# malani86/unet-DC-segmentation

Hardware: NVIDIA B200
Metric: images/sec end-to-end (mask + droplet table) (higher is better)
Workload: dtype bf16

## Files before the change

### include/unetdc_b200.h

```cpp
#ifndef UNETDC_B200_H
#define UNETDC_B200_H

#include <stddef.h>
#include <stdint.h>

#ifdef __cplusplus
extern "C" {
#endif

#define DC_OK 0
#define DC_EINVAL (-1)
#define DC_ECUDA (-2)
#define DC_EDEVICE (-3)
#define DC_ECAPACITY (-4)
#define DC_EWORKSPACE (-5)

#define DC_ABI_VERSION 205

const char* dc_last_error(void);
int dc_version(void);
int dc_device_check(int device, int* sm_count);

enum { DC_KIND_CONV3X3 = 0, DC_KIND_UPCONV2 = 1 };
enum {
    DC_EPI_STORE = 0,
    DC_EPI_STORE_POOL = 1,
    DC_EPI_HEAD = 2,
    DC_EPI_UPSCATTER = 3
};

typedef struct dc_conv_args {
    int kind;
    int epilogue;
    int relu;
    int B, H, W;
    int Cin, Cout;
    int dilation;
    const void* in;
    int in_stride;
    const void* weight;
    const float* bias;
    void* out;
    int out_stride;
    int out_offset;
    void* pool_out;
    int pool_stride;
    const float* head_w;
    float head_b;
    float thresh;
    float* prob_out;
    uint8_t* mask_out;
    const void* weight_par;
} dc_conv_args_t;

int dc_conv_tc(const dc_conv_args_t* args, void* stream);

typedef struct dc_upfuse_args {
    int B, H, W;
    const void* x;
    int x_stride;
    const void* skip;
    int skip_stride;
    const void* weight;
    const float* bias9;
    int relu;
    void* out;
    int out_stride;
    int out_offset;
    int channels;
    const void* weight_skip;
} dc_upfuse_args_t;

int dc_conv_upfused(const dc_upfuse_args_t* args, void* stream);
int dc_debug_upfuse_schedule(int* out, int cap);
int dc_debug_set_upfuse_mode(int mode);

enum { DC_CONV_FAMILY_AUTO = 0, DC_CONV_FAMILY_NO_PAIR = 1, DC_CONV_FAMILY_GENERIC = 2 };
int dc_debug_set_conv_family(int family);

typedef struct dc_stem_args {
    int in_kind;
    int B, H, W;
    int Cout;
    int dilation;
    const void* in;
    const float* weight;
    const float* bias;
    void* out;
    int out_stride;
    int out_offset;
} dc_stem_args_t;

int dc_stem(const dc_stem_args_t* args, void* stream);

typedef struct dc_model dc_model_t;

#define DC_NUM_LAYERS 23
typedef struct dc_model_desc {
    const void* weight[DC_NUM_LAYERS];
    const float* bias[DC_NUM_LAYERS];
    int dilations[5];
    int base_channels;
    int in_channels;
    int out_channels;
    const void* fused_weight1;
    const float* fused_bias1;
    const void* fused_wide_x[3];
    const void* fused_wide_s[3];
    const float* fused_wide_b[3];
    const void* par_weight[2];
} dc_model_desc_t;

int dc_model_create(dc_model_t** out, int device, const dc_model_desc_t* desc);
int dc_model_destroy(dc_model_t* m);
int dc_forward_workspace_bytes(const dc_model_t* m, int B, int H, int W, size_t* bytes);
int dc_forward(dc_model_t* m, int in_kind, const void* in, int B, int H, int W, float thresh, float* prob_out,
               uint8_t* mask_out, void* workspace, size_t workspace_bytes, void* stream);
int dc_forward_num_launches(const dc_model_t* m);
int dc_forward_profile(dc_model_t* m, int in_kind, const void* in, int B, int H, int W, float thresh, float* prob_out,
                       uint8_t* mask_out, void* workspace, size_t workspace_bytes, void* stream, float* launch_ms);

typedef struct dc_rolling_ball_args {
    const uint8_t* in;
    uint8_t* out;
    int B, H, W, C;
    int radius;
    void* workspace;
    size_t workspace_bytes;
} dc_rolling_ball_args_t;

// ... 96 lines not shown
```

### unet_dc_segmentation_b200/_lib.py

```python
from __future__ import annotations

import ctypes as C
from ctypes import POINTER, Structure, c_double, c_float, c_int, c_int32, c_int64, c_size_t, c_uint8, c_void_p

from . import build as _build

DC_OK = 0
DC_EINVAL, DC_ECUDA, DC_EDEVICE, DC_ECAPACITY, DC_EWORKSPACE = -1, -2, -3, -4, -5
DC_KIND_CONV3X3, DC_KIND_UPCONV2 = 0, 1
DC_EPI_STORE, DC_EPI_STORE_POOL, DC_EPI_HEAD, DC_EPI_UPSCATTER = 0, 1, 2, 3
DC_NUM_LAYERS = 23
DC_CONV_FAMILY_AUTO, DC_CONV_FAMILY_NO_PAIR, DC_CONV_FAMILY_GENERIC = 0, 1, 2
ABI_VERSION = 205

EXPORTS = [
    "dc_last_error", "dc_version", "dc_device_check", "dc_conv_tc", "dc_conv_upfused", "dc_debug_upfuse_schedule", "dc_debug_set_upfuse_mode", "dc_debug_set_conv_family", "dc_stem", "dc_model_create",
    "dc_model_destroy", "dc_forward_workspace_bytes", "dc_forward", "dc_forward_num_launches", "dc_forward_profile",
    "dc_rolling_ball_workspace_bytes", "dc_rolling_ball", "dc_rolling_ball_max_radius", "dc_debug_rolling_ball_plan", "dc_label_workspace_bytes", "dc_label_stats",
    "dc_resize_linear_u8", "dc_overlay_workspace_bytes", "dc_overlay_stencil",
    "dc_roi_workspace_bytes", "dc_roi_mask", "dc_radial_workspace_bytes", "dc_radial_density",
    "dc_spatial_workspace_bytes", "dc_spatial_density",
]


class DcError(RuntimeError):
    def __init__(self, code: int, msg: str):
        super().__init__(f"libunetdc_b200: {msg} (code {code})")
        self.code = code


class ConvArgs(Structure):
    _fields_ = [
        ("kind", c_int), ("epilogue", c_int), ("relu", c_int),
        ("B", c_int), ("H", c_int), ("W", c_int),
        ("Cin", c_int), ("Cout", c_int), ("dilation", c_int),
        ("in_", c_void_p), ("in_stride", c_int),
        ("weight", c_void_p), ("bias", c_void_p),
        ("out", c_void_p), ("out_stride", c_int), ("out_offset", c_int),
        ("pool_out", c_void_p), ("pool_stride", c_int),
        ("head_w", c_void_p), ("head_b", c_float), ("thresh", c_float),
        ("prob_out", c_void_p), ("mask_out", c_void_p),
        ("weight_par", c_void_p),
    ]


class StemArgs(Structure):
    _fields_ = [
        ("in_kind", c_int), ("B", c_int), ("H", c_int), ("W", c_int), ("Cout", c_int), ("dilation", c_int),
        ("in_", c_void_p), ("weight", c_void_p), ("bias", c_void_p), ("out", c_void_p),
        ("out_stride", c_int), ("out_offset", c_int),
    ]


class ModelDesc(Structure):
    _fields_ = [
        ("weight", c_void_p * DC_NUM_LAYERS), ("bias", c_void_p * DC_NUM_LAYERS),
        ("dilations", c_int * 5), ("base_channels", c_int), ("in_channels", c_int), ("out_channels", c_int),
        ("fused_weight1", c_void_p), ("fused_bias1", c_void_p),
        ("fused_wide_x", c_void_p * 3), ("fused_wide_s", c_void_p * 3), ("fused_wide_b", c_void_p * 3),
        ("par_weight", c_void_p * 2),
    ]


class UpfuseArgs(Structure):
    _fields_ = [
# ... 145 lines not shown
```

### unet_dc_segmentation_b200/csrc/conv_tc.cu

```cuda
#include "common.cuh"

#include <cuda.h>
#include <stdlib.h>
#include <string.h>

namespace dc {

namespace {

constexpr int TILE_H = 8, TILE_W = 16, TILE_M = TILE_H * TILE_W;
constexpr int KCHUNK = 64;
constexpr int A_STAGE_BYTES = TILE_M * KCHUNK * 2;
constexpr int NUM_THREADS = 384;
constexpr int EPI_WARP0 = 4;

int g_kernel_family = DC_CONV_FAMILY_AUTO;
int g_upfuse_mode = 0;

template <class K>
int set_max_smem_once(K kernel, int bytes, unsigned long long* done_mask) {
    int dev = 0;
    DC_CUDA(cudaGetDevice(&dev));
    const unsigned long long bit = 1ull << (dev & 63);
    if (!(__atomic_load_n(done_mask, __ATOMIC_ACQUIRE) & bit)) {
        DC_CUDA(cudaFuncSetAttribute(kernel, cudaFuncAttributeMaxDynamicSharedMemorySize, bytes));
        __atomic_fetch_or(done_mask, bit, __ATOMIC_RELEASE);
    }
    return DC_OK;
}

struct FastDiv {
    uint32_t mul, shift;
};
inline FastDiv make_fastdiv(int d) {
    FastDiv f;
    uint32_t s = 0;
    while ((1ll << s) < d) ++s;
    f.shift = 31 + s;
    f.mul = (uint32_t)(((1ull << f.shift) / (uint32_t)d) + 1ull);
    return f;
}
__device__ __forceinline__ int fast_div(int n, const FastDiv& f) {
    return (int)(((unsigned long long)(uint32_t)n * f.mul) >> f.shift);
}

struct alignas(64) ConvParams {
    CUtensorMap tmA;
    CUtensorMap tmB;
    CUtensorMap tmS;
    CUtensorMap tmB2;
    int B, H, W, Cin, Cout;
    int dil, ntaps, kchunks;
    int tiles_w, tiles_h, n_tiles, total_tiles, m_tiles;
    FastDiv fd_ntiles, fd_per_img, fd_tiles_w;
    int epilogue, relu;
    const float* bias;
    int bias_const;
    float bias_c[64];
    __nv_bfloat16* out;
    int out_stride, out_offset;
    __nv_bfloat16* pool_out;
    int pool_stride;
    const float* head_w;
    float head_b, thresh;
    float* prob_out;
    uint8_t* mask_out;
    int region_w, region_h, region_stride, nstages, nbstages;
    int border_bias;
    int real_ntiles;
};

struct TileCoord {
    int img, h0, w0, n0;
};

template <int TH = TILE_H, int TW = TILE_W>
__device__ __forceinline__ TileCoord decode_tile(const ConvParams& p, int tile, int BN) {
    TileCoord t;
    int m = fast_div(tile, p.fd_ntiles);
    int nt = tile - m * p.n_tiles;
    int per_img = p.tiles_h * p.tiles_w;
    t.img = fast_div(m, p.fd_per_img);
    int r = m - t.img * per_img;
    int th = fast_div(r, p.fd_tiles_w);
    t.h0 = th * TH;
    t.w0 = (r - th * p.tiles_w) * TW;
    t.n0 = nt * BN;
    return t;
}

template <int TH = TILE_H, int TW = TILE_W>
__device__ __forceinline__ bool tap_offset(const ConvParams& p, const TileCoord& t, int tap, int& dy, int& dx) {
    if (p.ntaps == 1) { dy = 0; dx = 0; return true; }
    int ky = tap / 3, kx = tap - ky * 3;
    dy = (ky - 1) * p.dil;
    dx = (kx - 1) * p.dil;
    return (t.h0 + dy + TH > 0) && (t.h0 + dy < p.H) && (t.w0 + dx + TW > 0) && (t.w0 + dx < p.W);
}

__device__ __forceinline__ uint32_t pack_bf16(float a, float b) {
    __nv_bfloat162 h = __floats2bfloat162_rn(a, b);
    return *reinterpret_cast<uint32_t*>(&h);
}
__device__ __forceinline__ uint32_t max_bf16x2(uint32_t a, uint32_t b) {
    __nv_bfloat162 r = __hmax2(*reinterpret_cast<__nv_bfloat162*>(&a), *reinterpret_cast<__nv_bfloat162*>(&b));
    return *reinterpret_cast<uint32_t*>(&r);
}

__device__ __forceinline__ int pair_count(const ConvParams& p) {
    return ((p.m_tiles + 1) >> 1) * p.n_tiles;
}
__device__ __forceinline__ int pair_to_tile(const ConvParams& p, int pair, int rank) {
    const int m_tiles = p.m_tiles;
    const int mpair = fast_div(pair, p.fd_ntiles), nt = pair - mpair * p.n_tiles;
    int m = 2 * mpair + rank;
    if (m >= m_tiles) m = m_tiles - 1;
    return m * p.n_tiles + nt;
}

__device__ __forceinline__ void tmem_ld_wait_on(uint32_t* v) {
    asm volatile("tcgen05.wait::ld.sync.aligned;"
                 : "+r"(v[0]), "+r"(v[1]), "+r"(v[2]), "+r"(v[3]), "+r"(v[4]), "+r"(v[5]), "+r"(v[6]), "+r"(v[7]),
                   "+r"(v[8]), "+r"(v[9]), "+r"(v[10]), "+r"(v[11]), "+r"(v[12]), "+r"(v[13]), "+r"(v[14]), "+r"(v[15]),
                   "+r"(v[16]), "+r"(v[17]), "+r"(v[18]), "+r"(v[19]), "+r"(v[20]), "+r"(v[21]), "+r"(v[22]), "+r"(v[23]),
                   "+r"(v[24]), "+r"(v[25]), "+r"(v[26]), "+r"(v[27]), "+r"(v[28]), "+r"(v[29]), "+r"(v[30]), "+r"(v[31])
                 :
                 : "memory");
}

constexpr int EPI_GROUPS = 2;
constexpr int EPI_STAGE_BYTES = 32 * 64;
constexpr int EPI_STAGE_TOTAL = EPI_GROUPS * 4 * EPI_STAGE_BYTES;

__device__ __forceinline__ uint32_t stg_off(int r, int q) {
    return (uint32_t)(((r >> 1) << 7) | (((r ^ (r >> 1)) & 1) << 6) | ((q ^ ((r >> 1) & 3)) << 4));
}

__device__ __forceinline__ uint32_t pack_bf16_relu(float a, float b) {
    uint32_t r;
    asm("cvt.rn.relu.bf16x2.f32 %0, %1, %2;" : "=r"(r) : "f"(b), "f"(a));
    return r;
}
template <bool PAIR>
__device__ __forceinline__ void release_accumulator(uint64_t* bar, int lane) {
    tc_fence_before();
    __syncwarp();
    if (lane == 0) {
        if (PAIR) mbar_arrive_leader(bar);
        else mbar_arrive(bar);
    }
}

template <int BN, int TH, int TW, int NHALF = 1, bool PAIR = false, bool COOP = true, bool UPF = false>
__device__ __forceinline__ void run_epilogue(const ConvParams& p, const int e, const int lane, const int group,
                                             const uint32_t tmem_base, uint64_t* tfull_bar, uint64_t* tempty_bar,
                                             const float* bias_s, uint8_t* stg_all) {
    const int L = e * 32 + lane;
    const int lh = L / TW, lw = L % TW;
    const float* head_s = bias_s + p.Cout;
    uint8_t* stg = stg_all + (group * 4 + e) * EPI_STAGE_BYTES;
    const int sq = lane & 3;
    const int pool_r0 = (TW == 16) ? 2 * (lane >> 2) : (16 * (lane >> 4) + 2 * ((lane >> 2) & 3));
    constexpr int CPG = COOP ? BN / 64 : BN / 32;
    constexpr int CSTEP = COOP ? 64 : 32;
    constexpr int NI = NHALF * CPG;
    const int cgrp = COOP ? group * 32 : 0;
    const bool up = !UPF && p.epilogue == DC_EPI_UPSCATTER;
// ... 265 lines not shown
                }
            }
        }
    } else if (warp == 1) {
        const uint32_t idesc = umma_idesc_bf16(TILE_M, BN);
        int stage = 0;
        uint32_t phase = 0;
        int it = 0;
        for (int tile = blockIdx.x; tile < p.total_tiles; tile += gridDim.x, ++it) {
            const TileCoord t = decode_tile(p, tile, BN);
            const int as = it & 1;
            const uint32_t aphase = (uint32_t)(it >> 1) & 1u;
            mbar_wait(&tempty_bar[as], aphase ^ 1u);
            tc_fence_after();
            const uint32_t d_tmem = tmem_base + (uint32_t)(as * BN);
            uint32_t accumulate = 0;
            for (int tap = 0; tap < p.ntaps; ++tap) {
                int dy, dx;
                if (!tap_offset(p, t, tap, dy, dx)) continue;
                for (int kc = 0; kc < p.kchunks; ++kc) {
                    mbar_wait(&full_bar[stage], phase);
                    tc_fence_after();
                    const uint32_t sa = smem_u32(smem + stage * STAGE_BYTES);
                    const uint64_t adesc = umma_desc_sw128(sa);
                    const uint64_t bdesc = umma_desc_sw128(sa + A_STAGE_BYTES);
                    if (elect_one()) {
#pragma unroll
                        for (int k = 0; k < KCHUNK / 16; ++k) {
                            umma_bf16(d_tmem, adesc + (uint64_t)(2 * k), bdesc + (uint64_t)(2 * k), idesc,
                                      (k == 0) ? accumulate : 1u);
                        }
                        umma_commit(&empty_bar[stage]);
                    }
                    __syncwarp();
                    accumulate = 1;
                    if (++stage == NSTAGES) { stage = 0; phase ^= 1u; }
                }
            }
            if (elect_one()) umma_commit(&tfull_bar[as]);
            __syncwarp();
        }
    } else if (warp >= EPI_WARP0) {
        run_epilogue<BN, TILE_H, TILE_W>(p, warp & 3, lane, (warp - EPI_WARP0) >> 2, tmem_base, tfull_bar, tempty_bar, bias_s, stg_s);
    }

    tc_fence_before();
    __syncthreads();
    if (warp == 2) {
        tc_fence_after();
        tmem_dealloc(tmem_base, TMEM_COLS);
    }
}

constexpr int HT_H = 16, HT_W = 8;
constexpr int HALO_MAX_STAGES = 8;
constexpr int HALO_BAR_BYTES = 512;
constexpr int HALO_BIAS_BYTES = 4096 + 256;

__device__ __forceinline__ uint64_t umma_desc_sw128_strided(uint32_t smem_addr, uint32_t sbo_bytes) {
    uint64_t d = 0;
    d |= (uint64_t)((smem_addr & 0x3FFFF) >> 4);
    d |= (uint64_t)1 << 16;
    d |= (uint64_t)((sbo_bytes >> 4) & 0x3FFF) << 32;
    d |= (uint64_t)1 << 46;
    d |= (uint64_t)2 << 61;
    return d;
}

template <int BN, int HT_NHALF, bool WRES>
__global__ void __launch_bounds__(NUM_THREADS, 1) conv_halo_kernel(const __grid_constant__ ConvParams p) {
    constexpr int HT_TW = HT_W * HT_NHALF;
    constexpr int W_TILE_BYTES = BN * KCHUNK * 2;
    constexpr int TMEM_COLS = 2 * HT_NHALF * BN;

    extern __shared__ uint8_t smem_raw[];
    uint8_t* smem = smem_raw + ((1024u - (smem_u32(smem_raw) & 1023u)) & 1023u);
    const int n_wtiles = WRES ? 9 * p.kchunks : p.nbstages;
    uint8_t* w_res = smem;
    uint8_t* a_ring = smem + n_wtiles * W_TILE_BYTES;
    uint64_t* full_bar = reinterpret_cast<uint64_t*>(a_ring + p.nstages * p.region_stride);
    uint64_t* empty_bar = full_bar + HALO_MAX_STAGES;
    uint64_t* bfull_bar = empty_bar + HALO_MAX_STAGES;
    uint64_t* bempty_bar = bfull_bar + HALO_MAX_STAGES;
    uint64_t* tfull_bar = bempty_bar + HALO_MAX_STAGES;
    uint64_t* tempty_bar = tfull_bar + 2;
    uint64_t* w_bar = tempty_bar + 2;
    uint32_t* tmem_slot = reinterpret_cast<uint32_t*>(w_bar + 1);
    float* bias_s = reinterpret_cast<float*>(reinterpret_cast<uint8_t*>(full_bar) + HALO_BAR_BYTES);
    uint8_t* stg_s = reinterpret_cast<uint8_t*>(full_bar) + HALO_BAR_BYTES + HALO_BIAS_BYTES;

    const int warp = threadIdx.x >> 5, lane = threadIdx.x & 31;
    const int NST = p.nstages;
    const int NBS = p.nbstages;

    stage_bias(p, bias_s);
    if (warp == 0 && lane == 0) {
        tma_prefetch_desc(&p.tmA);
        tma_prefetch_desc(&p.tmB);
    }
    if (warp == 1 && lane == 0) {
        for (int s = 0; s < HALO_MAX_STAGES; ++s) {
            mbar_init(&full_bar[s], 1); mbar_init(&empty_bar[s], 1);
            mbar_init(&bfull_bar[s], 1); mbar_init(&bempty_bar[s], 1);
        }
        for (int s = 0; s < 2; ++s) { mbar_init(&tfull_bar[s], 1); mbar_init(&tempty_bar[s], 4 * EPI_GROUPS); }
        mbar_init(w_bar, 1);
// ... 1084 lines not shown
    }

    tc_fence_before();
    __syncthreads();
    if (warp == 12) {
        tc_fence_after();
        tmem_dealloc(tmem_base, TMEM_COLS);
    }
}


typedef CUresult (*EncodeTiledFn)(CUtensorMap*, CUtensorMapDataType, cuuint32_t, void*, const cuuint64_t*,
                                  const cuuint64_t*, const cuuint32_t*, const cuuint32_t*, CUtensorMapInterleave,
                                  CUtensorMapSwizzle, CUtensorMapL2promotion, CUtensorMapFloatOOBfill);

EncodeTiledFn encode_fn() {
    static EncodeTiledFn fn = nullptr;
    if (!fn) {
        void* ptr = nullptr;
        cudaDriverEntryPointQueryResult qres;
        if (cudaGetDriverEntryPoint("cuTensorMapEncodeTiled", &ptr, cudaEnableDefault, &qres) == cudaSuccess &&
            qres == cudaDriverEntryPointSuccess)
            fn = reinterpret_cast<EncodeTiledFn>(ptr);
    }
    return fn;
}

int encode_map(CUtensorMap* m, const void* base, int rank, const cuuint64_t* dims, const cuuint64_t* strides_bytes,
               const cuuint32_t* box, CUtensorMapSwizzle swizzle = CU_TENSOR_MAP_SWIZZLE_128B) {
    EncodeTiledFn fn = encode_fn();
    DC_REQUIRE(fn, DC_ECUDA, "cuTensorMapEncodeTiled entry point not available");
    cuuint32_t estr[5] = {1, 1, 1, 1, 1};
    CUresult r = fn(m, CU_TENSOR_MAP_DATA_TYPE_BFLOAT16, (cuuint32_t)rank, const_cast<void*>(base), dims, strides_bytes,
                    box, estr, CU_TENSOR_MAP_INTERLEAVE_NONE, swizzle,
                    CU_TENSOR_MAP_L2_PROMOTION_L2_256B, CU_TENSOR_MAP_FLOAT_OOB_FILL_NONE);
    DC_REQUIRE(r == CUDA_SUCCESS, DC_ECUDA, "cuTensorMapEncodeTiled failed (CUresult %d)", (int)r);
    return DC_OK;
}

template <int BN, int NSTAGES>
int launch_variant(const ConvParams& p, cudaStream_t stream) {
    constexpr int STAGE_BYTES = A_STAGE_BYTES + BN * KCHUNK * 2;
    constexpr size_t SMEM = (size_t)NSTAGES * STAGE_BYTES + 1024  + 256  +
                            4096 + 256  + EPI_STAGE_TOTAL;
    static_assert(SMEM <= 227 * 1024, "stage ring exceeds shared memory");
    static unsigned long long attr_done = 0;
    { int rc = set_max_smem_once(conv_tc_kernel<BN, NSTAGES>, (int)SMEM, &attr_done); if (rc != DC_OK) return rc; }
    int grid = p.total_tiles < num_sms() ? p.total_tiles : num_sms();
    conv_tc_kernel<BN, NSTAGES><<<grid, NUM_THREADS, SMEM, stream>>>(p);
    DC_CUDA(cudaGetLastError());
    return DC_OK;
}

}

static int launch_conv_par(const dc_conv_args_t* a, cudaStream_t stream, const float* bias_host) {
    DC_REQUIRE(((uintptr_t)a->weight_par & 15) == 0, DC_EINVAL, "dc_conv_tc: weight_par must be 16-byte aligned");
    ConvParams p;
    memset(&p, 0, sizeof(p));
    const int Hh = a->H / 2, Wh = a->W / 2;
    {
        const cuuint64_t ps = (cuuint64_t)a->in_stride * 2;
        cuuint64_t dims[5] = {64, 2, (cuuint64_t)Wh, (cuuint64_t)a->H, (cuuint64_t)a->B};
        cuuint64_t str[4] = {ps, 2 * ps, (cuuint64_t)a->W * ps, (cuuint64_t)a->H * a->W * ps};
        cuuint32_t box[5] = {KCHUNK, 1, UPF_S_W, UPF_S_H, 1};
        int rc = encode_map(&p.tmS, a->in, 5, dims, str, box);
        if (rc != DC_OK) return rc;
    }
    {
        cuuint64_t dims[2] = {KCHUNK, (cuuint64_t)2 * PAR_ROWS_PER_RANK};
        cuuint64_t str[1] = {KCHUNK * 2};
        cuuint32_t box[2] = {KCHUNK, UPF_GROUP_ROWS};
        int rc = encode_map(&p.tmB, a->weight_par, 2, dims, str, box);
        if (rc != DC_OK) return rc;
    }
    p.B = a->B; p.H = Hh; p.W = Wh; p.Cin = 64; p.Cout = 64;
    p.dil = 1; p.ntaps = 9; p.kchunks = 1;
    p.tiles_w = ceil_div(Wh, HT_W);
    p.tiles_h = ceil_div(Hh, HT_H);
    p.n_tiles = 1;
    const long long total = (long long)a->B * p.tiles_w * p.tiles_h;
    DC_REQUIRE(total < (1ll << 31), DC_EINVAL, "dc_conv_tc: too many tiles");
    p.total_tiles = p.m_tiles = (int)total;
    p.fd_ntiles = make_fastdiv(1); p.fd_per_img = make_fastdiv(p.tiles_h * p.tiles_w); p.fd_tiles_w = make_fastdiv(p.tiles_w);
    p.epilogue = a->epilogue;
    p.relu = a->relu != 0;
    p.bias = a->bias;
    if (bias_host && a->epilogue != DC_EPI_HEAD) {
        p.bias_const = 1;
        memcpy(p.bias_c, bias_host, sizeof(p.bias_c));
    }
    p.out = reinterpret_cast<__nv_bfloat16*>(a->out);
    p.out_stride = a->out_stride; p.out_offset = a->out_offset;
    p.pool_out = reinterpret_cast<__nv_bfloat16*>(a->pool_out);
    p.pool_stride = a->pool_stride;
    p.head_w = a->head_w; p.head_b = a->head_b; p.thresh = a->thresh;
    p.prob_out = a->prob_out; p.mask_out = a->mask_out;

    const int n_pairs = (p.m_tiles + 1) / 2;
    const int max_clusters = num_sms() / 2;
    const int grid = 2 * (n_pairs < max_clusters ? n_pairs : max_clusters);
#define DC_PAR_CASE(mode)                                                                                    \
    if (g_upfuse_mode == mode) {                                                                             \
        static unsigned long long attr_done = 0;                                                             \
        int rc = set_max_smem_once(conv_par2_kernel<mode>, (int)PAR_SMEM, &attr_done);                       \
        if (rc != DC_OK) return rc;                                                                          \
        conv_par2_kernel<mode><<<grid, NUM_THREADS, PAR_SMEM, stream>>>(p);                                  \
    }
    DC_PAR_CASE(0) DC_PAR_CASE(1) DC_PAR_CASE(2) DC_PAR_CASE(3)
#undef DC_PAR_CASE
    DC_CUDA(cudaGetLastError());
    return DC_OK;
}

int launch_conv_tc(const dc_conv_args_t* a, cudaStream_t stream, const float* bias_host) {
    DC_REQUIRE(a && a->in && a->weight && a->bias, DC_EINVAL, "dc_conv_tc: null pointer argument");
    DC_REQUIRE(a->kind == DC_KIND_CONV3X3 || a->kind == DC_KIND_UPCONV2, DC_EINVAL, "dc_conv_tc: kind %d", a->kind);
    DC_REQUIRE(a->B > 0 && a->H > 0 && a->W > 0, DC_EINVAL, "dc_conv_tc: bad shape %d x %d x %d", a->B, a->H, a->W);
    DC_REQUIRE(a->Cin > 0 && a->Cin % KCHUNK == 0, DC_EINVAL, "dc_conv_tc: Cin %d must be a multiple of 64", a->Cin);
    DC_REQUIRE(a->Cout > 0 && a->Cout % 64 == 0 && a->Cout <= 1024, DC_EINVAL,
               "dc_conv_tc: Cout %d must be a multiple of 64 and at most 1024", a->Cout);
    DC_REQUIRE(a->in_stride >= a->Cin && a->in_stride % 8 == 0, DC_EINVAL, "dc_conv_tc: in_stride %d", a->in_stride);
    DC_REQUIRE(((uintptr_t)a->in & 15) == 0 && ((uintptr_t)a->weight & 15) == 0, DC_EINVAL,
               "dc_conv_tc: in / weight must be 16-byte aligned");
    const bool up = a->kind == DC_KIND_UPCONV2;
    DC_REQUIRE(up == (a->epilogue == DC_EPI_UPSCATTER), DC_EINVAL, "dc_conv_tc: kind %d with epilogue %d", a->kind,
               a->epilogue);
    DC_REQUIRE(a->epilogue >= DC_EPI_STORE && a->epilogue <= DC_EPI_UPSCATTER, DC_EINVAL, "dc_conv_tc: epilogue %d",
               a->epilogue);
    DC_REQUIRE(up || a->dilation >= 1, DC_EINVAL, "dc_conv_tc: dilation %d", a->dilation);
    if (a->epilogue == DC_EPI_HEAD) {
        DC_REQUIRE(a->Cout == 64 && a->head_w && (a->prob_out || a->mask_out), DC_EINVAL,
                   "dc_conv_tc: HEAD epilogue needs Cout == 64, head_w and prob_out or mask_out");
    } else {
        DC_REQUIRE(a->out && ((uintptr_t)a->out & 15) == 0, DC_EINVAL, "dc_conv_tc: out must be 16-byte aligned");
        DC_REQUIRE(a->out_stride % 8 == 0 && a->out_offset % 8 == 0 && a->out_offset >= 0 &&
                       a->out_stride >= a->out_offset + a->Cout,
                   DC_EINVAL, "dc_conv_tc: out_stride %d / out_offset %d", a->out_stride, a->out_offset);
    }
    if (a->epilogue == DC_EPI_STORE_POOL) {
        DC_REQUIRE(a->pool_out && ((uintptr_t)a->pool_out & 15) == 0 && a->pool_stride % 8 == 0 &&
                       a->pool_stride >= a->Cout,
                   DC_EINVAL, "dc_conv_tc: pool_out / pool_stride");
        DC_REQUIRE(a->H % 2 == 0 && a->W % 2 == 0, DC_EINVAL, "dc_conv_tc: pooled layer needs even H, W");
    }
    if (!up && a->weight_par && a->Cin == 64 && a->Cout == 64 && a->dilation == 1 && a->H % 2 == 0 && a->W % 2 == 0 &&
        g_kernel_family == DC_CONV_FAMILY_AUTO)
        return launch_conv_par(a, stream, bias_host);
    const int gemm_n = up ? 4 * a->Cout : a->Cout;
    const int BN = gemm_n % 256 == 0 ? 256 : (gemm_n % 128 == 0 ? 128 : 64);

    ConvParams p;
    memset(&p, 0, sizeof(p));

    bool halo = false, halo_wres = true, halo_pair = false;
    int halo_nhalf = 1;
    size_t halo_smem = 0;
    if (!up && a->dilation <= 4 && g_kernel_family == DC_CONV_FAMILY_AUTO) {
        const size_t w_tile = (size_t)(BN / 2) * KCHUNK * 2;
        const size_t w_half = (size_t)9 * (a->Cin / KCHUNK) * w_tile;
        const size_t budget = 227 * 1024 - 1024 - HALO_BAR_BYTES - HALO_BIAS_BYTES - EPI_STAGE_TOTAL;
        const int nh_max = BN == 256 ? 1 : (BN == 128 ? 2 : 4);
        for (int nh = nh_max; nh >= (BN == 64 ? 2 : nh_max) && !halo; --nh) {
        const int rw = HT_W * nh + 2 * a->dilation, rh = HT_H + 2 * a->dilation;
        const size_t region_stride = (size_t)rw * rh * KCHUNK * 2;
        for (int pass = 0; pass < 2 && !halo; ++pass) {
            size_t wsm = w_half;
            int nb = 0;
            if (pass == 0 && (a->Cout != BN || BN == 256)) continue;
            if (pass == 1) {
                if (BN == 64 || budget < 2 * region_stride + 4 * w_tile) break;
                nb = (int)((budget - 2 * region_stride) / w_tile);
                if (nb > HALO_MAX_STAGES) nb = HALO_MAX_STAGES;
                wsm = (size_t)nb * w_tile;
            }
            const long long nst = wsm < budget ? (long long)((budget - wsm) / region_stride) : 0;
            if (nst >= 2) {
                halo = halo_pair = true;
                halo_wres = pass == 0;
                halo_nhalf = nh;
                p.region_w = rw; p.region_h = rh; p.region_stride = (int)region_stride;
                p.nstages = nst > HALO_MAX_STAGES ? HALO_MAX_STAGES : (int)nst;
                p.nbstages = nb;
                halo_smem = wsm + (size_t)p.nstages * region_stride + 1024 + HALO_BAR_BYTES + HALO_BIAS_BYTES + EPI_STAGE_TOTAL;
            }
        }
        }
    }
    if (!halo && !up && a->Cout == BN && BN <= 128 && a->dilation <= 4) {
        const size_t w_tile = (size_t)BN * KCHUNK * 2;
        const size_t w_bytes = (size_t)9 * (a->Cin / KCHUNK) * w_tile;
        const size_t budget = 227 * 1024 - 1024  - HALO_BAR_BYTES - HALO_BIAS_BYTES -
                              EPI_STAGE_TOTAL ;
        static const int order128[4][2] = {{2, 0}, {2, 1}, {1, 0}, {1, 1}};
        static const int order64[4][2] = {{2, 0}, {1, 0}, {2, 1}, {1, 1}};
        for (int oi = 0; oi < 4 && !halo; ++oi) {
            {
                const int nhalf = (BN == 128 ? order128 : order64)[oi][0];
                const int pass = (BN == 128 ? order128 : order64)[oi][1];
                const int rw = HT_W * nhalf + 2 * a->dilation, rh = HT_H + 2 * a->dilation;
                const size_t region_stride = (size_t)rw * rh * KCHUNK * 2;
                size_t wsm = w_bytes;
                int nb = 0;
                if (pass == 1) {
                    if (budget < 2 * region_stride + 4 * w_tile) continue;
                    const size_t room = budget - 2 * region_stride;
                    nb = (int)(room / w_tile);
                    if (nb > HALO_MAX_STAGES) nb = HALO_MAX_STAGES;
                    wsm = (size_t)nb * w_tile;
                }
                const long long nst = wsm < budget ? (long long)((budget - wsm) / region_stride) : 0;
                if (nst >= 2) {
                    halo = true;
                    halo_wres = pass == 0;
                    halo_nhalf = nhalf;
                    p.region_w = rw; p.region_h = rh; p.region_stride = (int)region_stride;
                    p.nstages = nst > HALO_MAX_STAGES ? HALO_MAX_STAGES : (int)nst;
                    p.nbstages = nb;
                    halo_smem = wsm + (size_t)p.nstages * region_stride + 1024 + HALO_BAR_BYTES + HALO_BIAS_BYTES + EPI_STAGE_TOTAL;
                }
            }
        }
    }
    if (g_kernel_family == DC_CONV_FAMILY_GENERIC) halo = halo_pair = false;
    {
        cuuint64_t dims[4] = {(cuuint64_t)a->Cin, (cuuint64_t)a->W, (cuuint64_t)a->H, (cuuint64_t)a->B};
        cuuint64_t str[3] = {(cuuint64_t)a->in_stride * 2, (cuuint64_t)a->W * a->in_stride * 2,
                             (cuuint64_t)a->H * a->W * a->in_stride * 2};
        cuuint32_t box[4] = {KCHUNK, TILE_W, TILE_H, 1};
        if (halo) { box[1] = (cuuint32_t)p.region_w; box[2] = (cuuint32_t)p.region_h; }
        int rc = encode_map(&p.tmA, a->in, 4, dims, str, box);
        if (rc != DC_OK) return rc;
    }
    {
        const int ktot = up ? a->Cin : 9 * a->Cin;
        const int rows = up ? 4 * a->Cout : a->Cout;
        cuuint64_t dims[2] = {(cuuint64_t)ktot, (cuuint64_t)rows};
        cuuint64_t str[1] = {(cuuint64_t)ktot * 2};
        cuuint32_t box[2] = {KCHUNK, (cuuint32_t)(halo_pair ? BN / 2 : BN)};
        int rc = encode_map(&p.tmB, a->weight, 2, dims, str, box);
        if (rc != DC_OK) return rc;
    }
    p.B = a->B; p.H = a->H; p.W = a->W; p.Cin = a->Cin; p.Cout = a->Cout;
    p.dil = up ? 1 : a->dilation;
    p.ntaps = up ? 1 : 9;
    p.kchunks = a->Cin / KCHUNK;
    p.tiles_w = ceil_div(a->W, halo ? HT_W * halo_nhalf : TILE_W);
    p.tiles_h = ceil_div(a->H, halo ? HT_H : TILE_H);
    p.n_tiles = (up ? 4 * a->Cout : a->Cout) / BN;
    const long long total = (long long)a->B * p.tiles_w * p.tiles_h * p.n_tiles;
    DC_REQUIRE(total < (1ll << 31), DC_EINVAL, "dc_conv_tc: too many tiles");
    p.total_tiles = (int)total;
    p.m_tiles = p.total_tiles / p.n_tiles;
    p.fd_ntiles = make_fastdiv(p.n_tiles); p.fd_per_img = make_fastdiv(p.tiles_h * p.tiles_w); p.fd_tiles_w = make_fastdiv(p.tiles_w);
    p.epilogue = a->epilogue;
    p.relu = up ? 0 : (a->relu != 0);
    p.bias = a->bias;
    if (bias_host && a->Cout == 64 && a->epilogue != DC_EPI_HEAD) {
        p.bias_const = 1;
        memcpy(p.bias_c, bias_host, sizeof(p.bias_c));
    }
    p.out = reinterpret_cast<__nv_bfloat16*>(a->out);
    p.out_stride = a->out_stride; p.out_offset = a->out_offset;
    p.pool_out = reinterpret_cast<__nv_bfloat16*>(a->pool_out);
    p.pool_stride = a->pool_stride;
    p.head_w = a->head_w; p.head_b = a->head_b; p.thresh = a->thresh;
    p.prob_out = a->prob_out; p.mask_out = a->mask_out;

    if (halo_pair) {
        const int m_tiles = p.total_tiles / p.n_tiles;
        const int n_pairs = ((m_tiles + 1) / 2) * p.n_tiles;
        const int max_clusters = num_sms() / 2;
        const int grid = 2 * (n_pairs < max_clusters ? n_pairs : max_clusters);
#define DC_PAIR_CASE(bn, nh, wr)                                                                                      \
        if (BN == bn && halo_nhalf == nh && halo_wres == wr) {                                                        \
            static unsigned long long attr_done = 0;                                                                  \
            int rc_ = set_max_smem_once(conv_halo2_kernel<bn, nh, wr>, 227 * 1024, &attr_done);                       \
            if (rc_ != DC_OK) return rc_;                                                                             \
            conv_halo2_kernel<bn, nh, wr><<<grid, NUM_THREADS, halo_smem, stream>>>(p);                               \
        }
        DC_PAIR_CASE(64, 4, true) DC_PAIR_CASE(64, 3, true) DC_PAIR_CASE(64, 2, true)
        DC_PAIR_CASE(128, 2, true) DC_PAIR_CASE(128, 2, false) DC_PAIR_CASE(256, 1, false)
#undef DC_PAIR_CASE
        DC_CUDA(cudaGetLastError());
        return DC_OK;
    }
    if (halo) {
        const int grid = p.total_tiles < num_sms() ? p.total_tiles : num_sms();
#define DC_HALO_CASE(bn, nh, wr)                                                                                     \
        if (BN == bn && halo_nhalf == nh && halo_wres == wr) {                                                       \
            static unsigned long long attr_done = 0;                                                                 \
            int rc_ = set_max_smem_once(conv_halo_kernel<bn, nh, wr>, 227 * 1024, &attr_done);                       \
            if (rc_ != DC_OK) return rc_;                                                                            \
            conv_halo_kernel<bn, nh, wr><<<grid, NUM_THREADS, halo_smem, stream>>>(p);                               \
        }
        DC_HALO_CASE(64, 1, true) DC_HALO_CASE(64, 2, true) DC_HALO_CASE(128, 1, true) DC_HALO_CASE(128, 2, true)
        DC_HALO_CASE(64, 1, false) DC_HALO_CASE(64, 2, false) DC_HALO_CASE(128, 1, false) DC_HALO_CASE(128, 2, false)
#undef DC_HALO_CASE
        DC_CUDA(cudaGetLastError());
        return DC_OK;
    }
    switch (BN) {
        case 256: return launch_variant<256, 4>(p, stream);
        case 128: return launch_variant<128, 6>(p, stream);
        default:  return launch_variant<64, 8>(p, stream);
    }
}

static int launch_conv_upfused_wide(const dc_upfuse_args_t* a, cudaStream_t stream) {
    const int C = a->channels;
    const int BN = C == 128 ? 128 : 256;
    const int ncls = 256 / BN, groups = 4 / ncls, real_ntiles = C / BN, SC = C / KCHUNK;
    DC_REQUIRE(a->weight_skip && ((uintptr_t)a->weight_skip & 15) == 0, DC_EINVAL, "dc_conv_upfused: weight_skip");
    ConvParams p;
    memset(&p, 0, sizeof(p));
    {
        cuuint64_t dims[4] = {(cuuint64_t)2 * C, (cuuint64_t)a->W, (cuuint64_t)a->H, (cuuint64_t)a->B};
        cuuint64_t str[3] = {(cuuint64_t)a->x_stride * 2, (cuuint64_t)a->W * a->x_stride * 2,
                             (cuuint64_t)a->H * a->W * a->x_stride * 2};
        cuuint32_t box[4] = {KCHUNK, UPF_U_W, UPF_U_H, 1};
        int rc = encode_map(&p.tmA, a->x, 4, dims, str, box);
        if (rc != DC_OK) return rc;
    }
    {
        const cuuint64_t ps = (cuuint64_t)a->skip_stride * 2;
        cuuint64_t dims[5] = {(cuuint64_t)C, 2, (cuuint64_t)a->W, (cuuint64_t)(2 * a->H), (cuuint64_t)a->B};
        cuuint64_t str[4] = {ps, 2 * ps, 2 * (cuuint64_t)a->W * ps, 4 * (cuuint64_t)a->H * a->W * ps};
        cuuint32_t box[5] = {KCHUNK, 1, UPF_S_W, UPF_S_H, 1};
        int rc = encode_map(&p.tmS, a->skip, 5, dims, str, box);
        if (rc != DC_OK) return rc;
    }
    {
        cuuint64_t dims[2] = {KCHUNK, (cuuint64_t)groups * real_ntiles * 2 * (2 * SC) * 4 * UPF_GROUP_ROWS};
        cuuint64_t str[1] = {KCHUNK * 2};
        cuuint32_t box[2] = {KCHUNK, UPF_GROUP_ROWS};
        int rc = encode_map(&p.tmB, a->weight, 2, dims, str, box);
        if (rc != DC_OK) return rc;
    }
    {
        cuuint64_t dims[2] = {KCHUNK, (cuuint64_t)real_ntiles * 2 * SC * 9 * (BN / 2)};
        cuuint64_t str[1] = {KCHUNK * 2};
        cuuint32_t box[2] = {KCHUNK, (cuuint32_t)(BN / 2)};
        int rc = encode_map(&p.tmB2, a->weight_skip, 2, dims, str, box);
        if (rc != DC_OK) return rc;
    }
    p.B = a->B; p.H = a->H; p.W = a->W; p.Cin = 3 * C; p.Cout = C;
    p.dil = 1; p.ntaps = 9; p.kchunks = SC;
    p.tiles_w = ceil_div(a->W, HT_W);
    p.tiles_h = ceil_div(a->H, HT_H);
    p.n_tiles = groups * real_ntiles;
    p.real_ntiles = real_ntiles;
    const long long total = (long long)a->B * p.tiles_w * p.tiles_h * p.n_tiles;
    DC_REQUIRE(total < (1ll << 31), DC_EINVAL, "dc_conv_upfused: too many tiles");
    p.total_tiles = (int)total;
// ... 84 lines not shown
    p.out = reinterpret_cast<__nv_bfloat16*>(a->out);
    p.out_stride = a->out_stride; p.out_offset = a->out_offset;

    const int n_pairs = (p.m_tiles + 1) / 2;
    const int max_clusters = num_sms() / 2;
    const int grid = 2 * (n_pairs < max_clusters ? n_pairs : max_clusters);
#define DC_UPF_CASE(mode)                                                                                    \
    if (g_upfuse_mode == mode) {                                                                             \
        static unsigned long long attr_done = 0;                                                             \
        int rc = set_max_smem_once(conv_upfused2_kernel<mode>, (int)UPF_SMEM, &attr_done);                   \
        if (rc != DC_OK) return rc;                                                                          \
        conv_upfused2_kernel<mode><<<grid, NUM_THREADS, UPF_SMEM, stream>>>(p);                              \
    }
    DC_UPF_CASE(0) DC_UPF_CASE(1) DC_UPF_CASE(2) DC_UPF_CASE(3)
#undef DC_UPF_CASE
    DC_CUDA(cudaGetLastError());
    return DC_OK;
}

template <int MODE>
int upfuse_schedule_of(int* out, int cap) {
    const int nu = upf_u_count<MODE>(), ns = upf_s_count<MODE>();
    const int n = 2 * nu + ns;
    DC_REQUIRE(out && cap >= 5 * n, DC_EINVAL, "dc_debug_upfuse_schedule: need room for %d ints", 5 * n);
    int* o = out;
    for (int kc = 0; kc < 2; ++kc)
        for (int i = 0; i < nu; ++i) {
            const UpfOp op = upf_u_op<MODE>(i);
            *o++ = kc; *o++ = op.r; *o++ = op.c; *o++ = op.cls0; *o++ = op.ncls;
        }
    for (int i = 0; i < ns; ++i) {
        const UpfOp op = upf_s_op<MODE>(i);
        *o++ = 2; *o++ = op.r; *o++ = op.c; *o++ = op.cls0; *o++ = op.ncls;
    }
    return n;
}

int upfuse_schedule(int* out, int cap) {
    switch (g_upfuse_mode) {
        case 1: return upfuse_schedule_of<1>(out, cap);
        case 2: return upfuse_schedule_of<2>(out, cap);
        case 3: return upfuse_schedule_of<3>(out, cap);
        default: return upfuse_schedule_of<0>(out, cap);
    }
}

int set_upfuse_mode(int mode) {
    DC_REQUIRE(mode >= 0 && mode < UPF_MODES, DC_EINVAL, "dc_debug_set_upfuse_mode: %d", mode);
    g_upfuse_mode = mode;
    return DC_OK;
}

int set_conv_family(int family) {
    DC_REQUIRE(family >= DC_CONV_FAMILY_AUTO && family <= DC_CONV_FAMILY_GENERIC, DC_EINVAL, "dc_debug_set_conv_family: %d", family);
    g_kernel_family = family;
    return DC_OK;
}

int launch_stem(const dc_stem_args_t* a, cudaStream_t stream, const float* bias_host) {
    DC_REQUIRE(a && a->in && a->weight && a->bias && a->out, DC_EINVAL, "dc_stem: null pointer argument");
    DC_REQUIRE(a->Cout == 64, DC_EINVAL, "dc_stem: Cout must be 64 (got %d)", a->Cout);
    DC_REQUIRE(a->B > 0 && a->H > 0 && a->W > 0 && a->dilation >= 1, DC_EINVAL, "dc_stem: bad shape");
    DC_REQUIRE(a->out_stride % 8 == 0 && a->out_offset % 8 == 0 && a->out_stride >= a->out_offset + 64, DC_EINVAL,
               "dc_stem: output stride/offset must be multiples of 8 channels");
    DC_REQUIRE(((uintptr_t)a->out & 15) == 0, DC_EINVAL, "dc_stem: out must be 16-byte aligned");
    DC_REQUIRE(a->in_kind >= 0 && a->in_kind <= 2, DC_EINVAL, "dc_stem: in_kind %d", a->in_kind);
    StemParams sp;
    memset(&sp, 0, sizeof(sp));
    ConvParams& p = sp.c;
    p.B = a->B; p.H = a->H; p.W = a->W; p.Cin = 3; p.Cout = 64;
    p.dil = a->dilation; p.ntaps = 9; p.kchunks = 1;
    p.tiles_w = ceil_div(a->W, TILE_W);
    p.tiles_h = ceil_div(a->H, TILE_H);
    p.n_tiles = 1;
    const long long total = (long long)a->B * p.tiles_w * p.tiles_h;
    DC_REQUIRE(total < (1ll << 31), DC_EINVAL, "dc_stem: too many tiles");
    p.total_tiles = (int)total;
    p.m_tiles = p.total_tiles / p.n_tiles;
    p.fd_ntiles = make_fastdiv(p.n_tiles); p.fd_per_img = make_fastdiv(p.tiles_h * p.tiles_w); p.fd_tiles_w = make_fastdiv(p.tiles_w);
    p.epilogue = DC_EPI_STORE; p.relu = 1;
    p.bias = a->bias;
    if (bias_host) {
        p.bias_const = 1;
        memcpy(p.bias_c, bias_host, sizeof(p.bias_c));
    }
    p.out = reinterpret_cast<__nv_bfloat16*>(a->out);
    p.out_stride = a->out_stride; p.out_offset = a->out_offset;
    sp.in = a->in; sp.weight = a->weight; sp.in_kind = a->in_kind;
    {
        cuuint64_t dims[4] = {(cuuint64_t)a->out_stride, (cuuint64_t)a->W, (cuuint64_t)a->H, (cuuint64_t)a->B};
        cuuint64_t str[3] = {(cuuint64_t)a->out_stride * 2, (cuuint64_t)a->W * a->out_stride * 2,
                             (cuuint64_t)a->H * a->W * a->out_stride * 2};
        cuuint32_t box[4] = {32, TILE_W, 2, 1};
        int rc = encode_map(&p.tmA, a->out, 4, dims, str, box, CU_TENSOR_MAP_SWIZZLE_64B);
        if (rc != DC_OK) return rc;
    }
    constexpr size_t SMEM = 64 * 128 + (size_t)STEM_STAGES * A_STAGE_BYTES + 1024  +
                            1024  + STEM_STG_BYTES;
    static unsigned long long attr_done[3] = {0, 0, 0};
    {
        int rc = set_max_smem_once(stem_tc_kernel<0>, (int)SMEM, &attr_done[0]);
        if (rc == DC_OK) rc = set_max_smem_once(stem_tc_kernel<1>, (int)SMEM, &attr_done[1]);
        if (rc == DC_OK) rc = set_max_smem_once(stem_tc_kernel<2>, (int)SMEM, &attr_done[2]);
        if (rc != DC_OK) return rc;
    }
    const int grid = p.total_tiles < num_sms() ? p.total_tiles : num_sms();
    switch (a->in_kind) {
// ... 10 lines not shown
```

Baseline: 945.7.

## Add 2-SM cluster per-tap conv kernel pairing images for BN=256 layers

Adds a cta_group::2 tcgen05 conv kernel for non-halo, non-upconv layers with 256 output channels. The two CTAs of a cluster work on the same spatial tile in two different images and each loads half of the weight tile, so weight traffic and shared memory per CTA are halved. That frees room for 6 pipeline stages instead of 4 and allows M=256 MMAs. Pairing by image needs care with odd batch sizes (the last image is duplicated). A debug family value is added to turn the path off.

```diff
diff --git a/include/unetdc_b200.h b/include/unetdc_b200.h
--- a/include/unetdc_b200.h
+++ b/include/unetdc_b200.h
@@ -75,7 +75,7 @@
 int dc_debug_upfuse_schedule(int* out, int cap);
 int dc_debug_set_upfuse_mode(int mode);
 
-enum { DC_CONV_FAMILY_AUTO = 0, DC_CONV_FAMILY_NO_PAIR = 1, DC_CONV_FAMILY_GENERIC = 2 };
+enum { DC_CONV_FAMILY_AUTO = 0, DC_CONV_FAMILY_NO_PAIR = 1, DC_CONV_FAMILY_GENERIC = 2, DC_CONV_FAMILY_NO_PERTAP_PAIR = 3 };
 int dc_debug_set_conv_family(int family);
 
 typedef struct dc_stem_args {
diff --git a/unet_dc_segmentation_b200/_lib.py b/unet_dc_segmentation_b200/_lib.py
--- a/unet_dc_segmentation_b200/_lib.py
+++ b/unet_dc_segmentation_b200/_lib.py
@@ -10,7 +10,7 @@
 DC_KIND_CONV3X3, DC_KIND_UPCONV2 = 0, 1
 DC_EPI_STORE, DC_EPI_STORE_POOL, DC_EPI_HEAD, DC_EPI_UPSCATTER = 0, 1, 2, 3
 DC_NUM_LAYERS = 23
-DC_CONV_FAMILY_AUTO, DC_CONV_FAMILY_NO_PAIR, DC_CONV_FAMILY_GENERIC = 0, 1, 2
+DC_CONV_FAMILY_AUTO, DC_CONV_FAMILY_NO_PAIR, DC_CONV_FAMILY_GENERIC, DC_CONV_FAMILY_NO_PERTAP_PAIR = 0, 1, 2, 3
 ABI_VERSION = 205
 
 EXPORTS = [
diff --git a/unet_dc_segmentation_b200/csrc/conv_tc.cu b/unet_dc_segmentation_b200/csrc/conv_tc.cu
--- a/unet_dc_segmentation_b200/csrc/conv_tc.cu
+++ b/unet_dc_segmentation_b200/csrc/conv_tc.cu
@@ -68,6 +68,7 @@
     int region_w, region_h, region_stride, nstages, nbstages;
     int border_bias;
     int real_ntiles;
+    int pair_imgs;
 };
 
 struct TileCoord {
@@ -108,11 +109,19 @@
 }
 
 __device__ __forceinline__ int pair_count(const ConvParams& p) {
+    if (p.pair_imgs) return ((p.B + 1) >> 1) * (p.tiles_h * p.tiles_w) * p.n_tiles;
     return ((p.m_tiles + 1) >> 1) * p.n_tiles;
 }
 __device__ __forceinline__ int pair_to_tile(const ConvParams& p, int pair, int rank) {
+    const int mpair = fast_div(pair, p.fd_ntiles), nt = pair - mpair * p.n_tiles;
+    if (p.pair_imgs) {
+        const int per_img = p.tiles_h * p.tiles_w;
+        const int ipair = fast_div(mpair, p.fd_per_img), pos = mpair - ipair * per_img;
+        int img = 2 * ipair + rank;
+        if (img >= p.B) img = p.B - 1;
+        return (img * per_img + pos) * p.n_tiles + nt;
+    }
     const int m_tiles = p.m_tiles;
-    const int mpair = fast_div(pair, p.fd_ntiles), nt = pair - mpair * p.n_tiles;
     int m = 2 * mpair + rank;
     if (m >= m_tiles) m = m_tiles - 1;
     return m * p.n_tiles + nt;
@@ -484,6 +493,125 @@
     }
 }
 
+template <int BN, int NSTAGES>
+__global__ void __cluster_dims__(2, 1, 1) __launch_bounds__(NUM_THREADS, 1)
+conv_tc2_kernel(const __grid_constant__ ConvParams p) {
+    constexpr int B_STAGE_BYTES = (BN / 2) * KCHUNK * 2;
+    constexpr int STAGE_BYTES = A_STAGE_BYTES + B_STAGE_BYTES;
+    constexpr int TMEM_COLS = 2 * BN;
+    static_assert(TMEM_COLS <= 512, "accumulators exceed TMEM");
+
+    extern __shared__ uint8_t smem_raw[];
+    uint8_t* smem = smem_raw + ((1024u - (smem_u32(smem_raw) & 1023u)) & 1023u);
+    uint64_t* full_bar = reinterpret_cast<uint64_t*>(smem + NSTAGES * STAGE_BYTES);
+    uint64_t* empty_bar = full_bar + NSTAGES;
+    uint64_t* tfull_bar = empty_bar + NSTAGES;
+    uint64_t* tempty_bar = tfull_bar + 2;
+    uint32_t* tmem_slot = reinterpret_cast<uint32_t*>(tempty_bar + 2);
+    float* bias_s = reinterpret_cast<float*>(smem + NSTAGES * STAGE_BYTES + 256);
+    uint8_t* stg_s = smem + NSTAGES * STAGE_BYTES + 256 + 4096 + 256;
+
+    const int warp = threadIdx.x >> 5, lane = threadIdx.x & 31;
+    const uint32_t rank = cluster_ctarank();
+    const bool leader = rank == 0;
+    const int cluster_id = blockIdx.x >> 1, n_clusters = gridDim.x >> 1;
+    const int n_pairs = pair_count(p);
+
+    stage_bias(p, bias_s);
+    if (warp == 0 && lane == 0) {
+        tma_prefetch_desc(&p.tmA);
+        tma_prefetch_desc(&p.tmB);
+    }
+    if (warp == 1 && lane == 0) {
+        for (int s = 0; s < NSTAGES; ++s) { mbar_init(&full_bar[s], 1); mbar_init(&empty_bar[s], 1); }
+        for (int s = 0; s < 2; ++s) { mbar_init(&tfull_bar[s], 1); mbar_init(&tempty_bar[s], 8 * EPI_GROUPS); }
+        fence_barrier_init();
+    }
+    if (warp == 2) {
+        tmem_alloc_2sm(tmem_slot, TMEM_COLS);
+        tmem_relinquish_2sm();
+    }
+    tc_fence_before();
+    __syncthreads();
+    cluster_sync_all();
+    tc_fence_after();
+    const uint32_t tmem_base = *tmem_slot;
+
+    if (warp == 0) {
+        int stage = 0;
+        uint32_t phase = 0;
+        for (int pair = cluster_id; pair < n_pairs; pair += n_clusters) {
+            const TileCoord t = decode_tile(p, pair_to_tile(p, pair, (int)rank), BN);
+            for (int tap = 0; tap < p.ntaps; ++tap) {
+                int dy, dx;
+                if (!tap_offset(p, t, tap, dy, dx)) continue;
+                for (int kc = 0; kc < p.kchunks; ++kc) {
+                    mbar_wait(&empty_bar[stage], phase ^ 1u);
+                    if (elect_one()) {
+                        uint8_t* sa = smem + stage * STAGE_BYTES;
+                        if (leader) mbar_expect_tx(&full_bar[stage], 2 * STAGE_BYTES);
+                        tma_load_4d_2sm(sa, &p.tmA, &full_bar[stage], kc * KCHUNK, t.w0 + dx, t.h0 + dy, t.img);
+                        tma_load_2d_2sm(sa + A_STAGE_BYTES, &p.tmB, &full_bar[stage], tap * p.Cin + kc * KCHUNK,
+                                        t.n0 + (int)rank * (BN / 2));
+                    }
+                    __syncwarp();
+                    if (++stage == NSTAGES) { stage = 0; phase ^= 1u; }
+                }
+            }
+        }
+    } else if (warp == 1) {
+        if (leader) {
+            const uint32_t idesc = umma_idesc_bf16(2 * TILE_M, BN);
+            int stage = 0;
+            uint32_t phase = 0;
+            int it = 0;
+            for (int pair = cluster_id; pair < n_pairs; pair += n_clusters, ++it) {
+                const TileCoord t = decode_tile(p, pair_to_tile(p, pair, 0), BN);
+                const int as = it & 1;
+                const uint32_t aphase = (uint32_t)(it >> 1) & 1u;
+                mbar_wait(&tempty_bar[as], aphase ^ 1u);
+                tc_fence_after();
+                const uint32_t d_tmem = tmem_base + (uint32_t)(as * BN);
+                uint32_t accumulate = 0;
+                for (int tap = 0; tap < p.ntaps; ++tap) {
+                    int dy, dx;
+                    if (!tap_offset(p, t, tap, dy, dx)) continue;
+                    for (int kc = 0; kc < p.kchunks; ++kc) {
+                        mbar_wait(&full_bar[stage], phase);
+                        tc_fence_after();
+                        const uint32_t sa = smem_u32(smem + stage * STAGE_BYTES);
+                        const uint64_t adesc = umma_desc_sw128(sa);
+                        const uint64_t bdesc = umma_desc_sw128(sa + A_STAGE_BYTES);
+                        if (elect_one()) {
+#pragma unroll
+                            for (int k = 0; k < KCHUNK / 16; ++k)
+                                umma_bf16_2sm(d_tmem, adesc + (uint64_t)(2 * k), bdesc + (uint64_t)(2 * k), idesc,
+                                              (k == 0) ? accumulate : 1u);
+                            umma_commit_2sm(&empty_bar[stage]);
+                        }
+                        __syncwarp();
+                        accumulate = 1;
+                        if (++stage == NSTAGES) { stage = 0; phase ^= 1u; }
+                    }
+                }
+                if (elect_one()) umma_commit_2sm(&tfull_bar[as]);
+                __syncwarp();
+            }
+        }
+    } else if (warp >= EPI_WARP0) {
+        run_epilogue<BN, TILE_H, TILE_W, 1, true>(p, warp & 3, lane, (warp - EPI_WARP0) >> 2, tmem_base, tfull_bar, tempty_bar,
+                                                  bias_s, stg_s);
+    }
+
+    tc_fence_before();
+    __syncthreads();
+    cluster_sync_all();
+    if (warp == 2) {
+        tc_fence_after();
+        tmem_dealloc_2sm(tmem_base, TMEM_COLS);
+    }
+}
+
 constexpr int HT_H = 16, HT_W = 8;
 constexpr int HALO_MAX_STAGES = 8;
 constexpr int HALO_BAR_BYTES = 512;
@@ -1674,6 +1802,22 @@
     return DC_OK;
 }
 
+template <int BN, int NSTAGES>
+int launch_variant2(const ConvParams& p, cudaStream_t stream) {
+    constexpr int STAGE_BYTES = A_STAGE_BYTES + (BN / 2) * KCHUNK * 2;
+    constexpr size_t SMEM = (size_t)NSTAGES * STAGE_BYTES + 1024  + 256  +
+                            4096 + 256  + EPI_STAGE_TOTAL;
+    static_assert(SMEM <= 227 * 1024, "stage ring exceeds shared memory");
+    static unsigned long long attr_done = 0;
+    { int rc = set_max_smem_once(conv_tc2_kernel<BN, NSTAGES>, (int)SMEM, &attr_done); if (rc != DC_OK) return rc; }
+    const int n_pairs = ((p.B + 1) / 2) * p.tiles_h * p.tiles_w * p.n_tiles;
+    const int max_clusters = num_sms() / 2;
+    const int grid = 2 * (n_pairs < max_clusters ? n_pairs : max_clusters);
+    conv_tc2_kernel<BN, NSTAGES><<<grid, NUM_THREADS, SMEM, stream>>>(p);
+    DC_CUDA(cudaGetLastError());
+    return DC_OK;
+}
+
 }
 
 static int launch_conv_par(const dc_conv_args_t* a, cudaStream_t stream, const float* bias_host) {
@@ -1766,8 +1910,9 @@
                    DC_EINVAL, "dc_conv_tc: pool_out / pool_stride");
         DC_REQUIRE(a->H % 2 == 0 && a->W % 2 == 0, DC_EINVAL, "dc_conv_tc: pooled layer needs even H, W");
     }
+    const bool auto_family = g_kernel_family == DC_CONV_FAMILY_AUTO || g_kernel_family == DC_CONV_FAMILY_NO_PERTAP_PAIR;
     if (!up && a->weight_par && a->Cin == 64 && a->Cout == 64 && a->dilation == 1 && a->H % 2 == 0 && a->W % 2 == 0 &&
-        g_kernel_family == DC_CONV_FAMILY_AUTO)
+        auto_family)
         return launch_conv_par(a, stream, bias_host);
     const int gemm_n = up ? 4 * a->Cout : a->Cout;
     const int BN = gemm_n % 256 == 0 ? 256 : (gemm_n % 128 == 0 ? 128 : 64);
@@ -1778,7 +1923,7 @@
     bool halo = false, halo_wres = true, halo_pair = false;
     int halo_nhalf = 1;
     size_t halo_smem = 0;
-    if (!up && a->dilation <= 4 && g_kernel_family == DC_CONV_FAMILY_AUTO) {
+    if (!up && a->dilation <= 4 && auto_family) {
         const size_t w_tile = (size_t)(BN / 2) * KCHUNK * 2;
         const size_t w_half = (size_t)9 * (a->Cin / KCHUNK) * w_tile;
         const size_t budget = 227 * 1024 - 1024 - HALO_BAR_BYTES - HALO_BIAS_BYTES - EPI_STAGE_TOTAL;
@@ -1845,6 +1990,7 @@
         }
     }
     if (g_kernel_family == DC_CONV_FAMILY_GENERIC) halo = halo_pair = false;
+    const bool pertap_pair = !up && !halo && BN == 256 && g_kernel_family == DC_CONV_FAMILY_AUTO;
     {
         cuuint64_t dims[4] = {(cuuint64_t)a->Cin, (cuuint64_t)a->W, (cuuint64_t)a->H, (cuuint64_t)a->B};
         cuuint64_t str[3] = {(cuuint64_t)a->in_stride * 2, (cuuint64_t)a->W * a->in_stride * 2,
@@ -1859,7 +2005,7 @@
         const int rows = up ? 4 * a->Cout : a->Cout;
         cuuint64_t dims[2] = {(cuuint64_t)ktot, (cuuint64_t)rows};
         cuuint64_t str[1] = {(cuuint64_t)ktot * 2};
-        cuuint32_t box[2] = {KCHUNK, (cuuint32_t)(halo_pair ? BN / 2 : BN)};
+        cuuint32_t box[2] = {KCHUNK, (cuuint32_t)(halo_pair || pertap_pair ? BN / 2 : BN)};
         int rc = encode_map(&p.tmB, a->weight, 2, dims, str, box);
         if (rc != DC_OK) return rc;
     }
@@ -1922,6 +2068,10 @@
         DC_CUDA(cudaGetLastError());
         return DC_OK;
     }
+    if (pertap_pair) {
+        p.pair_imgs = 1;
+        return launch_variant2<256, 6>(p, stream);
+    }
     switch (BN) {
         case 256: return launch_variant<256, 4>(p, stream);
         case 128: return launch_variant<128, 6>(p, stream);
@@ -2112,7 +2262,7 @@
 }
 
 int set_conv_family(int family) {
-    DC_REQUIRE(family >= DC_CONV_FAMILY_AUTO && family <= DC_CONV_FAMILY_GENERIC, DC_EINVAL, "dc_debug_set_conv_family: %d", family);
+    DC_REQUIRE(family >= DC_CONV_FAMILY_AUTO && family <= DC_CONV_FAMILY_NO_PERTAP_PAIR, DC_EINVAL, "dc_debug_set_conv_family: %d", family);
     g_kernel_family = family;
     return DC_OK;
 }
```

Result: faster. 955.3 (median of 6 runs) (+1.0%).
